# fhausmann/deepgrp

Measured on NVIDIA B200. Metric: bases classified/sec (Mbp/s): value = record resident in HBM (device-timed); e2e = FASTA text in host memory -> TSV text in host memory, higher is better.
Workload: dtype f32

## Files before the change

### deepgrp_b200/csrc/api.cu

```cuda
#include <math.h>
#include <stdarg.h>
#include <string.h>

#include <algorithm>
#include <chrono>
#include <condition_variable>
#include <deque>
#include <mutex>
#include <thread>

#include <cuda_fp16.h>
#include <cmath>

#include "dgrp_internal.cuh"

namespace dgrp {

static thread_local char g_err[1024] = "";

void set_error(const char *fmt, ...) {
  va_list ap;
  va_start(ap, fmt);
  vsnprintf(g_err, sizeof g_err, fmt, ap);
  va_end(ap);
// ... 247 lines not shown
  return DGRP_OK;
}

int dgrp_ctx_synchronize(dgrp_ctx *c) {
  Use use(c->device);
  DGRP_CUDA(cudaStreamSynchronize(c->stream));
  return DGRP_OK;
}
void *dgrp_ctx_stream(dgrp_ctx *c) { return (void *)c->stream; }
int dgrp_ctx_timings(dgrp_ctx *c, dgrp_timings_t *out) { *out = c->timings; return DGRP_OK; }
int64_t dgrp_ctx_launch_count(dgrp_ctx *c) { return c->launches; }

int dgrp_ctx_set_int(dgrp_ctx *c, const char *key, int64_t value) {
  if (!strcmp(key, "mss_chunk")) c->mss_chunk = (int)value;
  else if (!strcmp(key, "mss_max_rounds")) c->mss_max_rounds = (int)value;
  else if (!strcmp(key, "forward_tc")) c->forward_tc = (int)value;
  else if (!strcmp(key, "forward_sum16")) c->forward_sum16 = (int)value;
  else if (!strcmp(key, "forward_fp16x2")) c->forward_fp16x2 = (int)value;
  else if (!strcmp(key, "forward_gather")) c->forward_gather = (int)value;
  else if (!strcmp(key, "forward_fuse_score")) c->forward_fuse_score = (int)value;
  else if (!strcmp(key, "forward_smem_vote")) c->forward_smem_vote = (int)value;
  else if (!strcmp(key, "forward_wide")) c->forward_wide = (int)value;
  else if (!strcmp(key, "forward_overlap")) c->forward_overlap = (int)value;
  else if (!strcmp(key, "forward_ub")) c->forward_ub = (int)value;
  else if (!strcmp(key, "stream_slot_mb")) c->stream_slot_mb = (int)value;
  else if (!strcmp(key, "stream_early_rows")) c->stream_early_rows = (int)value;
  else if (!strcmp(key, "stream_early_slabs")) c->stream_early_slabs = (int)value;
  else if (!strcmp(key, "stream_early_unit")) c->stream_early_unit = (int)value;
  else if (!strcmp(key, "stream_early_ratio")) c->stream_early_ratio = (int)value;
  else if (!strcmp(key, "forward_slab_mb")) c->forward_slab_bytes = (int64_t)value << 20;
  else if (!strcmp(key, "shard_rank")) c->shard_rank = (int)value;
  else if (!strcmp(key, "shard_world")) c->shard_world = (int)value;
  else { set_error("unknown option %s", key); return DGRP_E_ARG; }
  return DGRP_OK;
}
int dgrp_ctx_get_int(dgrp_ctx *c, const char *key, int64_t *value) {
  if (!strcmp(key, "mss_chunk")) *value = c->mss_chunk;
  else if (!strcmp(key, "mss_max_rounds")) *value = c->mss_max_rounds;
  else if (!strcmp(key, "mss_rounds")) *value = c->mss_rounds;
  else if (!strcmp(key, "forward_tc")) *value = c->forward_tc;
  else if (!strcmp(key, "forward_sum16")) *value = c->forward_sum16;
  else if (!strcmp(key, "forward_fp16x2")) *value = c->forward_fp16x2;
  else if (!strcmp(key, "forward_gather")) *value = c->forward_gather;
  else if (!strcmp(key, "forward_fuse_score")) *value = c->forward_fuse_score;
  else if (!strcmp(key, "forward_smem_vote")) *value = c->forward_smem_vote;
  else if (!strcmp(key, "fused_last")) *value = c->fused_last;
  else if (!strcmp(key, "forward_wide")) *value = c->forward_wide;
  else if (!strcmp(key, "forward_overlap")) *value = c->forward_overlap;
  else if (!strcmp(key, "forward_ub")) *value = c->forward_ub;
  else if (!strcmp(key, "stream_slot_mb")) *value = c->stream_slot_mb;
  else if (!strcmp(key, "stream_early_rows")) *value = c->stream_early_rows;
  else if (!strcmp(key, "stream_early_slabs")) *value = c->stream_early_slabs;
  else if (!strcmp(key, "stream_early_unit")) *value = c->stream_early_unit;
  else if (!strcmp(key, "stream_early_ratio")) *value = c->stream_early_ratio;
  else if (!strcmp(key, "stream_early_parts")) *value = c->stream_early_parts;
  else if (!strcmp(key, "forward_slab_mb")) *value = c->forward_slab_bytes >> 20;
  else if (!strcmp(key, "forward_used_tc")) *value = c->forward_used_tc;
  else if (!strcmp(key, "sm_count")) *value = c->sm_count;
  else { set_error("unknown option %s", key); return DGRP_E_ARG; }
  return DGRP_OK;
}


int dgrp_one_hot_stage(dgrp_ctx *c, const uint8_t *seq, int64_t n, int fold_case,
                       int64_t *startpos, int64_t *out_len) {
  Use use(c->device);
  DGRP_REQUIRE(n >= 0, "negative length");
  c->staged_len = -1;
  DGRP_CHECK(c->raw.reserve((size_t)n + 16));
  if (n > 0) DGRP_CUDA(cudaMemcpyAsync(c->raw.p, seq, (size_t)n, cudaMemcpyHostToDevice, c->stream));
  DGRP_CHECK(c->small.reserve(256));
  DGRP_CHECK(c->pin_small.reserve(256));
  int64_t *d_fl = c->small.as<int64_t>() + 16;
  DGRP_CHECK(launch_trim(c, c->raw.as<uint8_t>(), n, fold_case, d_fl));
  int64_t *h = c->pin_small.as<int64_t>() + 8;
  DGRP_CUDA(cudaMemcpyAsync(h, d_fl, 16, cudaMemcpyDeviceToHost, c->stream));
  DGRP_CUDA(cudaStreamSynchronize(c->stream));
  *startpos = h[0];
  *out_len = h[1] - h[0];
  c->staged_n = n; c->staged_start = h[0]; c->staged_len = *out_len;
// ... 1440 lines not shown
```

### deepgrp_b200/csrc/dgrp_internal.cuh

```cuda
#pragma once
#include <cuda_runtime.h>
#include <stdint.h>
#include <stdio.h>
#include <string>
#include <utility>
#include <vector>

#include "../../include/deepgrp_b200.h"

namespace dgrp {

void set_error(const char *fmt, ...);

#define DGRP_CUDA(call)                                                                      \
  do {                                                                                       \
    cudaError_t e__ = (call);                                                                \
    if (e__ != cudaSuccess) {                                                                \
      dgrp::set_error("%s:%d: %s -> %s", __FILE__, __LINE__, #call, cudaGetErrorString(e__)); \
      return DGRP_E_CUDA;                                                                    \
    }                                                                                        \
  } while (0)

#define DGRP_CHECK(call)          \
  do {                            \
// ... 64 lines not shown
      io_a, io_b, io_c, small, segs, rows, mss_a, mss_b, mss_c, mss_d, mss_e, scan, winprobs, gapfill;
  dgrp::PinBuf pin_small, pin_a, pin_b;
  int mss_chunk = 0;
  int mss_max_rounds = 0;
  int mss_rounds = 0;
  int forward_tc = 1;
  int forward_sum16 = 1;
  int forward_fp16x2 = 1;
  int forward_gather = 1;
  int forward_wide = 0;
  int stream_slot_mb = 0;
  int stream_early_rows = 1;
  int stream_early_slabs = 0;
  int stream_early_unit = 0;
  int stream_early_ratio = 0;
  int stream_early_parts = 0;
  int forward_ub = 0;
  int forward_overlap = 1;
  int64_t forward_slab_bytes = (int64_t)8 << 30;
  int forward_smem_vote = 1;
  int forward_fuse_score = 1;
  int fused_last = 0;
  int forward_used_tc = 0;
  std::vector<dgrp_row_t> fa_rows;
  std::vector<int64_t> fa_hdr_off, fa_hdr_len, fa_startpos, fa_length, fa_tsv_off, fa_tsv_len, fa_owner;
  int64_t codes_dev_length = -1, codes_dev_rows = 0;
  uint64_t codes_dev_reserves[2] = {};
  int shard_rank = 0, shard_world = 1;
  dgrp::PinBuf tsv_host;
  int64_t tsv_len = 0;
  dgrp::DevBuf tsv_dev, tsv_prefix;
  dgrp::DevBuf st_raw[2], st_text[2];
  dgrp::PinBuf st_stage[2], st_slot[4];
  int64_t staged_n = 0, staged_start = 0, staged_len = -1;
};

namespace dgrp {

struct Use {
  int prev = -1;
  explicit Use(int dev) {
    cudaGetDevice(&prev);
    if (prev != dev) cudaSetDevice(dev);
    else prev = -1;
  }
  ~Use() {
// ... 58 lines not shown
```

### deepgrp_b200/csrc/forward.cu

```cuda
#include "forward_common.cuh"

namespace dgrp {

Placement make_placement(int64_t length, int T, int step, int batch_size, int compat) {
  Placement p;
  p.step = step;
  const int64_t W = length > T ? (length - T + step - 1) / step : 0;
  p.n_windows = W;
  p.full_windows = W;
  p.tail_base = 0;
  if (compat == DGRP_COMPAT_REFERENCE && batch_size > 0 && W % batch_size != 0) {
    const int64_t nb = W / batch_size, b_last = W % batch_size;
    p.full_windows = nb * batch_size;
    p.tail_base = nb * b_last * (int64_t)step;
  }
  return p;
}


int launch_forward_tc(dgrp_ctx *c, dgrp_model *m, FwdParams &p);
int launch_forward_tcw(dgrp_ctx *c, dgrp_model *m, FwdParams &p, int which);

template <int UP, int RNN = 0>
struct Cfg {
// ... 248 lines not shown

int run_forward_vote(dgrp_ctx *c, dgrp_model *m, const uint8_t *d_codes, int64_t codes_base,
                     int64_t w_begin, int64_t w_end, const Placement &pl, float *d_pred,
                     int64_t pred_row0, int64_t pred_rows, uint8_t *d_label, float *d_score, bool *fused,
                     int64_t w2_begin, int64_t w2_end) {
  if (fused) *fused = false;
  bool has2 = w2_end > w2_begin;
  if (has2 && w_end <= w_begin) { w_begin = w2_begin; w_end = w2_end; has2 = false; }
  auto second = [&]() -> int {
    return has2 ? run_forward_vote(c, m, d_codes, codes_base, w2_begin, w2_end, pl, d_pred, pred_row0, pred_rows) : DGRP_OK;
  };
  FwdParams p = {};
  fill_model(p, m);
  p.codes = d_codes; p.codes_base = codes_base;
  p.w_begin = w_begin; p.w_end = w_end;
  p.step = pl.step; p.full_windows = pl.full_windows; p.tail_base = pl.tail_base;
  p.pred = d_pred; p.pred_row0 = pred_row0; p.pred_rows = pred_rows;
  if (w_end <= w_begin) {
    if (fused && pred_rows > 0)
      DGRP_CUDA(cudaMemsetAsync(d_pred, 0, (size_t)pred_rows * m->C * sizeof(float), c->stream));
    return DGRP_OK;
  }
  c->forward_used_tc = 0;
  if (c->forward_tc) {
    auto dispatch = [&](FwdParams &q, int *used) -> int {
      int rc = DGRP_E_UNSUPPORTED;
      if (c->forward_wide == 0) { rc = launch_forward_tc(c, m, q); *used = 1; }
      if (rc == DGRP_E_UNSUPPORTED && c->forward_wide != 2) { rc = launch_forward_tcw(c, m, q, 1); *used = 2; }
      if (rc == DGRP_E_UNSUPPORTED) { rc = launch_forward_tcw(c, m, q, 2); *used = 3; }
      return rc;
    };
    bool smem_vote = false;
    if (w_end > w_begin) {
      FwdParams q = p;
      q.query = 1;
      int used = 0;
      smem_vote = dispatch(q, &used) == DGRP_OK && q.smem_vote;
    }
    const int64_t per_win = (int64_t)m->T * m->C * (int64_t)sizeof(float);
    int64_t slab = c->forward_slab_bytes / per_win;
    slab = slab < 4096 ? 4096 : slab & ~(int64_t)4095;
    p.win_probs = nullptr;
    if (c->forward_gather && !smem_vote) {
      const int64_t nw = w_end - w_begin < slab ? w_end - w_begin : slab;
      if (nw > 0 && c->winprobs.reserve((size_t)(nw * per_win)) == DGRP_OK) p.win_probs = c->winprobs.as<float>();
      else cudaGetLastError();
// ... 73 lines not shown
```

### deepgrp_b200/csrc/forward_tc.cu

```cuda
#include "forward_tc_common.cuh"

namespace dgrp {

template <int UP, int NP>
struct TCfg {
  static constexpr int NG = 3 * UP;
  static constexpr int N = 3 * UP + 16;
  static constexpr int ROWS = 128, WT = 64;
  static constexpr int UPT = UP / 4;
  static constexpr bool FOLD = NP == 2;
  static constexpr int KP = UP + (FOLD ? 16 : 0);
  static constexpr int KC = KP / 8;
  static constexpr int SBO = KC * 128;
  static constexpr int A_BYTES = ROWS * KP * 2;
  static constexpr int B_BYTES = N * KP * 2;
  static constexpr int PSTRIDE = 3 * UP + 4;
  static constexpr int TCOLS = N <= 64 ? 64 : (N <= 128 ? 128 : 256);
};


template <int UP, typename ST, int NP>
__global__ void __launch_bounds__(TC_THREADS, 1) gru_tc_attention_vote_kernel(const FwdParams p) {
  using K = TCfg<UP, NP>;
  extern __shared__ __align__(128) unsigned char smem_raw[];
  unsigned char *s_B = smem_raw;
  unsigned char *s_A = s_B + NP * K::B_BYTES;
  float *s_P = reinterpret_cast<float *>(s_A + 2 * NP * K::A_BYTES);
  float *s_bh = s_P + 10 * K::PSTRIDE;
  float *s_scale = s_bh + UP;
  float *s_score = s_scale + UP;
  uint8_t *s_codes = reinterpret_cast<uint8_t *>(s_score + (size_t)p.wpp * p.T);
  __shared__ __align__(8) unsigned long long s_ready[2], s_done[2];
  __shared__ uint32_t s_tmem;

  const int tid = threadIdx.x, lane = tid & 31, warp = tid >> 5;
  const int T = p.T;

  {
    const uint4 *src = reinterpret_cast<const uint4 *>(p.Bsplit);
    uint4 *dst = reinterpret_cast<uint4 *>(s_B);
    for (int i = tid; i < NP * K::B_BYTES / 16; i += TC_THREADS) dst[i] = src[i];
    for (int i = tid; i < 10 * K::PSTRIDE; i += TC_THREADS) {
      const int row = i / K::PSTRIDE, j = i % K::PSTRIDE;
      const int c = row >= 8 ? 4 : (row >= 4 ? 7 - row : row);
      float v = 0.f;
      if (j < 2 * UP) v = (p.P[c * 3 * UP + j] + p.b1[j]) * kNegLog2e;
      else if (j < 3 * UP) v = p.P[c * 3 * UP + j] * kTwoLog2e;
      s_P[i] = v;
    }
    for (int i = tid; i < UP; i += TC_THREADS) {
      s_bh[i] = p.b1[2 * UP + i] * kTwoLog2e;
      s_scale[i] = (p.attention && i < p.U) ? p.scale[i] : 0.f;
    }
  }
  if (warp == 0) {
    asm volatile("tcgen05.alloc.cta_group::1.sync.aligned.shared::cta.b32 [%0], %1;" ::"r"(
                     smem_u32(&s_tmem)),
                 "r"(2 * K::TCOLS)
                 : "memory");
    asm volatile("tcgen05.relinquish_alloc_permit.cta_group::1.sync.aligned;" ::: "memory");
  }
#ifdef DGRP_TC_TRACE
  for (int i = tid; i < 17 * 2 * 8; i += TC_THREADS) (&s_tc_trace[0][0][0])[i] = 0u;
  for (int i = tid; i < 16 * 8; i += TC_THREADS) (&s_tc_trace2[0][0])[i] = 0u;
#endif
  if (tid == 0) {
    mbar_init(smem_u32(&s_ready[0]), TC_GATE_WARPS * 32);
    mbar_init(smem_u32(&s_ready[1]), TC_GATE_WARPS * 32);
    mbar_init(smem_u32(&s_done[0]), 1);
    mbar_init(smem_u32(&s_done[1]), 1);
    asm volatile("fence.mbarrier_init.release.cluster;" ::: "memory");
  }
  fence_async_smem();
  tc_fence_before();
  __syncthreads();
  tc_fence_after();
  const uint32_t tmem_base = s_tmem;
  const bool is_gate = warp < TC_GATE_WARPS;
  const int extra = (T & 1) ? 0 : 1;
  const uint32_t bar_ready = smem_u32(&s_ready[0]), bar_done = smem_u32(&s_done[0]);
  const int64_t n_tiles = launch_tiles(p, K::WT);
  const int64_t tile_lo = n_tiles * blockIdx.x / gridDim.x, tile_hi = n_tiles * (blockIdx.x + 1) / gridDim.x;
  const int64_t my_tiles = tile_hi - tile_lo;
  const int lead = my_tiles >= 32 ? (int)(blockIdx.x & 3) : (my_tiles >= 16 ? (int)(blockIdx.x & 1) : 0);
  const uint32_t ab_fmt = NP == 3 ? 1u : 0u;
  const uint32_t idesc = (1u << 4) | (ab_fmt << 7) | (ab_fmt << 10) | ((uint32_t)(K::N >> 3) << 17) |
                         ((uint32_t)(128 >> 4) << 24);

  if (!is_gate) {
    asm volatile("setmaxnreg.dec.sync.aligned.u32 %0;" ::"n"(TC_AUX_REGS));
    if (warp != TC_GATE_WARPS) return;
    int unit = 0;
    for (int64_t tile = tile_lo; tile < tile_hi; ++unit) {
      const int nt = (unit < lead || tile + 1 >= tile_hi) ? 1 : 2;
      const bool live1 = nt == 2;
      TC_TRACE_DECL;
      for (int k = 0; k <= T + extra; ++k) {
#pragma unroll
        for (int s = 0; s < 2; ++s) {
          if (s == 1 && !live1) continue;
          TC_TRACE(6);
          mbar_wait_backoff(bar_ready + 8 * s, (uint32_t)(k & 1));
          tc_fence_after();
          TC_TRACE(5);
          if (lane == 0) {
            const uint32_t a0 = smem_u32(s_A + (size_t)s * NP * K::A_BYTES), b0 = smem_u32(s_B);
            const uint32_t d = tmem_base + (uint32_t)(s * K::TCOLS);
            const int pa[6] = {NP == 3 ? 2 : 1, 0, NP == 3 ? 1 : 0, 1, 0, 0};
            const int pb[6] = {0, NP == 3 ? 2 : 1, NP == 3 ? 1 : 0, 0, 1, 0};
            uint32_t acc = 0;
#pragma unroll
            for (int q = 0; q < (NP == 3 ? 6 : 3); ++q) {
              const int nkc = UP / 16 + ((K::FOLD && pa[q] == 0) ? 1 : 0);
#pragma unroll
              for (int kc = 0; kc < UP / 16 + 1; ++kc) {
                if (kc >= nkc) break;
                const uint64_t ad = umma_desc(a0 + pa[q] * K::A_BYTES + kc * 256, 128, K::SBO);
                const uint64_t bd = umma_desc(b0 + pb[q] * K::B_BYTES + kc * 256, 128, K::SBO);
                umma_bf16(d, ad, bd, idesc, acc);
                acc = 1;
              }
            }
            umma_commit(bar_done + 8 * s);
          }
          __syncwarp();
        }
      }
      tile += nt;
    }
#ifdef DGRP_TC_TRACE
    __syncwarp();
    if (blockIdx.x == 0 && lane < 16) g_tc_trace[16][lane >> 3][lane & 7] += s_tc_trace[16][lane >> 3][lane & 7];
#endif
    return;
  }

  asm volatile("setmaxnreg.inc.sync.aligned.u32 %0;" ::"n"(TC_GATE_REGS));
  ST *sum0 = reinterpret_cast<ST *>(p.scratch) + (size_t)blockIdx.x * 2 * K::WT * T * UP;
  float *proj0 = p.ff2 + (size_t)blockIdx.x * 2 * K::WT * T * 16;
  float *q0 = p.qbuf + (size_t)blockIdx.x * 2 * K::WT * UP;
  const float2 us = make_float2(p.b_unscale, p.b_unscale);
  int unit = 0;
  for (int64_t tile = tile_lo; tile < tile_hi; ++unit) {
    const int nt = (unit < lead || tile + 1 >= tile_hi) ? 1 : 2;
    const bool live1 = nt == 2;
    {
    const int quad = warp & 3, uq = warp >> 2;
    const int row = quad * 32 + lane;
    const int wl = row >> 1, dir = row & 1;
    const float *tblp = s_P + uq * K::UPT;
    const float *bhp = s_bh + uq * K::UPT;
    const uint32_t a_off = (uint32_t)((row >> 3) * K::SBO + (row & 7) * 16 + ((uq * K::UPT) >> 3) * 128);
    const size_t sum_thr = ((size_t)(wl / p.wpp) * T * (UP / 8) * p.wpp + (size_t)(wl % p.wpp)) * 8 + (dir ? 4 : 0);
    const uint32_t oh_off = (uint32_t)((row >> 3) * K::SBO + (row & 7) * 16 + (UP / 8) * 128);
    const uint32_t t_lane = tmem_base + ((uint32_t)(quad * 32) << 16);
    const int full_span = (K::WT - 1) * p.step + T;
    const int cbase = dir * p.code_span + (dir ? full_span - wl * p.step - T : wl * p.step);
    {
      const int nthr = TC_GATE_WARPS * 32;
      for (int s = 0; s < nt; ++s) {
        const TileRange tr = tile_range(p, tile + s, K::WT);
        const int64_t w_first = tr.w0;
        int64_t w_last = w_first + K::WT - 1;
        w_last = w_last < tr.hi ? w_last : tr.hi - 1;
        const int span = (int)((w_last - w_first) * p.step) + T;
        const uint8_t *src = p.codes + (w_first * (int64_t)p.step - p.codes_base);
        uint8_t *fwd_copy = s_codes + (size_t)(2 * s) * p.code_span, *rc_copy = fwd_copy + p.code_span;
        for (int i = tid; i < full_span; i += nthr) {
// ... 128 lines not shown
        }
        TC_TRACE(6);
      }
    }
#pragma unroll
    for (int s = 0; s < 2; ++s) {
      if (s == 1 && !live1) continue;
      mbar_wait(bar_done + 8 * s, (uint32_t)((T + extra) & 1));
      tc_fence_after();
      float pj[4];
      tmem_ld4(t_lane + (uint32_t)(s * K::TCOLS + K::NG + 4 * uq), pj);
      tmem_ld_wait();
      float4 o;
      o.x = pj[0] + __shfl_xor_sync(0xffffffffu, pj[0], 1);
      o.y = pj[1] + __shfl_xor_sync(0xffffffffu, pj[1], 1);
      o.z = pj[2] + __shfl_xor_sync(0xffffffffu, pj[2], 1);
      o.w = pj[3] + __shfl_xor_sync(0xffffffffu, pj[3], 1);
      if (NP == 2) { o.x *= us.x; o.y *= us.x; o.z *= us.x; o.w *= us.x; }
      if (dir == 0)
        *reinterpret_cast<float4 *>(proj0 + ((size_t)(s * K::WT + wl) * T + (T - 1)) * 16 + 4 * uq) = o;
    }
    tc_fence_before();
    }
    __threadfence_block();
    gate_bar_sync();
#pragma unroll 1
    for (int s = 0; s < nt; ++s)
      attention_vote_sum_tile<UP, K::WT, TC_GATE_WARPS, ST>(
          p, sum0 + (size_t)s * K::WT * T * UP, q0 + (size_t)s * K::WT * UP,
          proj0 + (size_t)s * K::WT * T * 16, tile_range(p, tile + s, K::WT), p.wpp, s_scale, s_score,
          p.smem_vote == 1 ? reinterpret_cast<float *>(s_A)
                           : (p.smem_vote == 2 ? reinterpret_cast<float *>(s_codes + 4 * (size_t)p.code_span) : nullptr));
    tile += nt;
  }

  tc_fence_before();
  gate_bar_sync();
#ifdef DGRP_TC_TRACE
  if (blockIdx.x == 0 && tid < 16 * 16) g_tc_trace[tid >> 4][(tid >> 3) & 1][tid & 7] += s_tc_trace[tid >> 4][(tid >> 3) & 1][tid & 7];
  if (blockIdx.x == 0 && tid < 16 * 8) g_tc_trace2[tid >> 3][tid & 7] += s_tc_trace2[tid >> 3][tid & 7];
#endif
  if (warp == 0) {
    asm volatile("tcgen05.dealloc.cta_group::1.sync.aligned.b32 %0, %1;" ::"r"(tmem_base),
                 "r"(2 * K::TCOLS)
                 : "memory");
  }
// ... 2 lines not shown
template <int UP, int NP>
static size_t tc_smem_bytes(int T, int wpp, int code_span) {
  using K = TCfg<UP, NP>;
  return (size_t)NP * K::B_BYTES + 2 * NP * K::A_BYTES +
         sizeof(float) * ((size_t)10 * K::PSTRIDE + 2 * UP + (size_t)wpp * T) + 4 * (size_t)code_span + 128;
}

template <int UP, typename ST, int NP>
static int launch_tc_t(dgrp_ctx *c, dgrp_model *m, FwdParams &p) {
  using K = TCfg<UP, NP>;
  const int64_t n_windows = p.w_end - p.w_begin;
  if (n_windows <= 0 && p.w2_end <= p.w2_begin) return DGRP_OK;
  const int64_t span = (int64_t)(K::WT - 1) * p.step + p.T;
  if (span > 16384) return DGRP_E_UNSUPPORTED;
  p.code_span = (int)((span + 15) & ~(int64_t)15);
  int wpp = K::WT;
  while (wpp > 8 && tc_smem_bytes<UP, NP>(p.T, wpp, p.code_span) > 227 * 1024) wpp >>= 1;
  const size_t smem = tc_smem_bytes<UP, NP>(p.T, wpp, p.code_span);
  if (smem > 227 * 1024) return DGRP_E_UNSUPPORTED;
  p.wpp = wpp;
  const size_t vote_bytes = (size_t)span * p.C * sizeof(float);
  size_t smem_total = smem;
  p.smem_vote = 0;
  if (c->forward_smem_vote) {
    if (vote_bytes <= (size_t)2 * NP * K::A_BYTES) p.smem_vote = 1;
    else if (smem + vote_bytes <= 227 * 1024) { p.smem_vote = 2; smem_total = smem + vote_bytes; }
  }
  if (p.query) return DGRP_OK;
  if (p.smem_vote) p.win_probs = nullptr;
  auto kern = gru_tc_attention_vote_kernel<UP, ST, NP>;
  DGRP_CUDA(cudaFuncSetAttribute(kern, cudaFuncAttributeMaxDynamicSharedMemorySize, (int)smem_total));
  const int64_t n_tiles = (n_windows > 0 ? (n_windows + K::WT - 1) / K::WT : 0) +
                          (p.w2_end > p.w2_begin ? (p.w2_end - p.w2_begin + K::WT - 1) / K::WT : 0);
  const int64_t n_pairs = (n_tiles + 1) / 2;
  const int grid = (int)(n_pairs < c->sm_count ? n_pairs : c->sm_count);
  const size_t rows = (size_t)grid * 2 * K::WT;
  DGRP_CHECK(c->avg.reserve(rows * p.T * UP * sizeof(ST) + rows * UP * sizeof(float)));
  DGRP_CHECK(c->io_c.reserve(rows * p.T * 16 * sizeof(float)));
  p.scratch = c->avg.as<float>();
  p.qbuf = reinterpret_cast<float *>(c->avg.as<unsigned char>() + rows * p.T * UP * sizeof(ST));
  p.ff2 = c->io_c.as<float>();
  kern<<<grid, TC_THREADS, smem_total, c->stream>>>(p);
  c->launches++;
  DGRP_CUDA(cudaGetLastError());
  return DGRP_OK;
}

#ifdef DGRP_TC_TRACE
extern "C" int dgrp_debug_tc_trace(unsigned long long *out, int reset) {
  if (reset) {
    static unsigned long long zero[17][2][8];
    return (int)cudaMemcpyToSymbol(g_tc_trace, zero, sizeof(zero));
  }
  return (int)cudaMemcpyFromSymbol(out, g_tc_trace, sizeof(unsigned long long) * 17 * 2 * 8);
}
extern "C" int dgrp_debug_tc_trace2(unsigned long long *out, int reset) {
  if (reset) {
    static unsigned long long zero[16][8];
    return (int)cudaMemcpyToSymbol(g_tc_trace2, zero, sizeof(zero));
  }
  return (int)cudaMemcpyFromSymbol(out, g_tc_trace2, sizeof(unsigned long long) * 16 * 8);
}
#endif

template <int UP>
static int launch_tc_up(dgrp_ctx *c, dgrp_model *m, FwdParams &p) {
// ... 18 lines not shown
```

### deepgrp_b200/csrc/forward_tc_common.cuh

```cuda
#pragma once
#include <cuda_bf16.h>
#include <cuda_fp16.h>

#include "forward_common.cuh"

namespace dgrp {

constexpr int TC_GATE_WARPS = 16;
constexpr int TC_THREADS = (TC_GATE_WARPS + 4) * 32;
constexpr int TC_GATE_REGS = 112, TC_AUX_REGS = 24;
constexpr float kNegLog2e = -1.4426950408889634f;
constexpr float kTwoLog2e = 2.8853900817779268f;

#ifdef DGRP_TC_TRACE
static __device__ unsigned long long g_tc_trace[17][2][8];
__shared__ unsigned int s_tc_trace[17][2][8];
#define TC_TRACE_DECL unsigned int tr_t = (unsigned int)clock64()
#define TC_TRACE(seg)                                                         \
  do {                                                                        \
    const unsigned int now__ = (unsigned int)clock64();                       \
    if (lane == 0) atomicAdd(&s_tc_trace[warp][s][seg], now__ - tr_t);        \
    tr_t = now__;                                                             \
  } while (0)
#define TC_TRACE2(seg)                                                        \
  do {                                                                        \
    const unsigned int now__ = (unsigned int)clock64();                       \
    if (lane == 0) atomicAdd(&s_tc_trace2[warp][seg], now__ - tr_t);          \
    tr_t = now__;                                                             \
  } while (0)
__shared__ unsigned int s_tc_trace2[16][8];
static __device__ unsigned long long g_tc_trace2[16][8];
#else
#define TC_TRACE_DECL
// ... 189 lines not shown
}
__device__ __forceinline__ void ldg256(const float *p, float (&v)[8]) {
  asm volatile("ld.global.v8.f32 {%0,%1,%2,%3,%4,%5,%6,%7}, [%8];"
               : "=f"(v[0]), "=f"(v[1]), "=f"(v[2]), "=f"(v[3]), "=f"(v[4]), "=f"(v[5]), "=f"(v[6]), "=f"(v[7])
               : "l"(p));
}
__device__ __forceinline__ float tanh_mufu(float x) {
  float y;
  asm("tanh.approx.f32 %0, %1;" : "=f"(y) : "f"(x));
  return y;
}
__device__ __forceinline__ float exp_fast(float x) {
  return ex2_approx(x * 1.4426950408889634f);
}
__device__ __forceinline__ float inv4_dot(const float *d, const float *sc) {
  const float2 d01 = make_float2(d[0], d[1]), d23 = make_float2(d[2], d[3]);
  const float2 m = __fmul2_rn(d01, d23);
  const float inv = rcp_approx(m.x * m.y);
  const float2 j = make_float2(inv * m.y, inv * m.x);
  const float2 i01 = __fmul2_rn(j, d23), i23 = __fmul2_rn(j, d01);
  return fmaf(sc[0], i01.x, fmaf(sc[1], i01.y, fmaf(sc[2], i23.x, sc[3] * i23.y)));
}

template <int UP, int WT, int NWARPS, typename ST>
__device__ __forceinline__ void attention_vote_sum_tile(const FwdParams &p, const ST *sum, const float *qbuf,
                                                        const float *proj, const TileRange tr, int wpp,
                                                        const float *s_scale, float *s_score, float *s_vote = nullptr) {
  const int64_t w_tile0 = tr.w0;
  const int tid = threadIdx.x, warp = tid >> 5, lane = tid & 31;
  const int T = p.T, C = p.C;
  const int vspan = (WT - 1) * p.step + T;
  if (s_vote) {
    for (int i = tid; i < vspan * C; i += NWARPS * 32) s_vote[i] = 0.f;
  }
  constexpr int NCH = UP / 8;
  constexpr int CPL = NCH / 4;
  constexpr int CH = CPL > 2 ? 2 : CPL;
  constexpr bool H16 = sizeof(ST) == 2;
  constexpr int NV = H16 ? 1 : 2;
  constexpr int UNR = H16 ? 4 : 2;
  constexpr int PU = 11;
  TC_TRACE_DECL;
  for (int w0 = 0; w0 < WT; w0 += wpp) {
    if (w_tile0 + w0 >= tr.hi) break;
    if (p.attention) {
      const int ngrp = wpp >> 3, grp = warp % ngrp, sl = warp / ngrp, nsl = NWARPS / ngrp;
      const int wi = lane & 7, cj = lane >> 3;
      const int wl = w0 + grp * 8 + wi;
      const int t_begin = (int)((int64_t)T * sl / nsl), t_end = (int)((int64_t)T * (sl + 1) / nsl);
#pragma unroll 1
      for (int i0 = 0; i0 < CPL; i0 += CH) {
      float q2[CH][8], sc2[CH][8];
#pragma unroll
      for (int i = 0; i < CH; ++i) {
        const int u0 = (cj + 4 * (i0 + i)) * 8;
#pragma unroll
        for (int j = 0; j < 8; ++j) {
          q2[i][j] = H16 ? qbuf[(size_t)wl * UP + u0 + j] : qbuf[(size_t)wl * UP + u0 + j] * kTwoLog2e;
          sc2[i][j] = H16 ? s_scale[u0 + j] : -2.0f * s_scale[u0 + j];
        }
      }
      const ST *sum_pass = sum + (size_t)(w0 / wpp) * T * NCH * wpp * 8;
      const ST *base = sum_pass + ((size_t)(cj + 4 * i0) * wpp + (grp * 8 + wi)) * 8;
      constexpr int PF_BLOCK = 4, PF_AHEAD = 12;
      const uint32_t ROW_BYTES = (uint32_t)(NCH * wpp * 8 * sizeof(ST));
      if (grp == 0 && lane == 0 && i0 == 0) {
        const int n0 = min(PF_AHEAD, t_end - t_begin);
        l2_prefetch(sum_pass + (size_t)t_begin * NCH * wpp * 8, (uint32_t)n0 * ROW_BYTES);
      }
      for (int t0 = t_begin; t0 < t_end; t0 += UNR) {
        if (grp == 0 && lane == 0 && i0 == 0 && (t0 - t_begin) % PF_BLOCK == 0) {
          const int ta = t0 + PF_AHEAD;
          if (ta < t_end) l2_prefetch(sum_pass + (size_t)ta * NCH * wpp * 8, (uint32_t)min(PF_BLOCK, t_end - ta) * ROW_BYTES);
        }
        uint4 v[UNR][CH][NV];
#pragma unroll
        for (int k = 0; k < UNR; ++k) {
          const int t = min(t0 + k, t_end - 1);
#pragma unroll
          for (int i = 0; i < CH; ++i)
#pragma unroll
            for (int n = 0; n < NV; ++n)
              v[k][i][n] = __ldcs(reinterpret_cast<const uint4 *>(base + ((size_t)t * NCH + 4 * i) * wpp * 8) + n);
        }
#pragma unroll
        for (int k = 0; k < UNR; ++k) {
          float sacc = 0.f;
#pragma unroll
          for (int i = 0; i < CH; ++i) {
            float x[8];
            if (H16) {
              const uint32_t wv[4] = {v[k][i][0].x, v[k][i][0].y, v[k][i][0].z, v[k][i][0].w};
#pragma unroll
              for (int j = 0; j < 4; ++j) {
                const float2 f = __half22float2(*reinterpret_cast<const __half2 *>(&wv[j]));
                x[2 * j] = f.x; x[2 * j + 1] = f.y;
              }
            } else {
              const uint32_t wv[8] = {v[k][i][0].x, v[k][i][0].y, v[k][i][0].z, v[k][i][0].w,
                                      v[k][i][NV - 1].x, v[k][i][NV - 1].y, v[k][i][NV - 1].z, v[k][i][NV - 1].w};
#pragma unroll
              for (int j = 0; j < 8; ++j) x[j] = __uint_as_float(wv[j]);
            }
            if (H16) {
#pragma unroll
              for (int j = 0; j < 8; ++j) sacc = fmaf(sc2[i][j], tanh_mufu(fmaf(x[j], 0.5f, q2[i][j])), sacc);
            } else {
              float d[8];
#pragma unroll
              for (int j = 0; j < 8; ++j)
                d[j] = ex2_approx(fminf(fmaf(x[j], 1.4426950408889634f, q2[i][j]), 30.0f)) + 1.0f;
              sacc += inv4_dot(d, sc2[i]) + inv4_dot(d + 4, sc2[i] + 4);
            }
          }
          sacc += __shfl_xor_sync(0xffffffffu, sacc, 8);
          sacc += __shfl_xor_sync(0xffffffffu, sacc, 16);
          if (cj == 0 && t0 + k < t_end) {
            float *dst = s_score + (size_t)(grp * 8 + wi) * T + t0 + k;
            *dst = (CH < CPL && i0 > 0) ? *dst + sacc : sacc;
          }
        }
      }
      }
    }
    if (lane == 0 && warp < wpp) l2_prefetch(proj + (size_t)(w0 + warp) * T * 16, (uint32_t)T * 64u);
    TC_TRACE2(0);
    asm volatile("bar.sync 1, %0;" ::"n"(NWARPS * 32) : "memory");
    TC_TRACE2(1);
    for (int wq = warp; wq < wpp; wq += NWARPS) {
      const int wl = w0 + wq;
      if (lane == 0 && wq + NWARPS < wpp)
        l2_prefetch(proj + (size_t)(wl + NWARPS) * T * 16, (uint32_t)T * 64u);
      const int64_t w = w_tile0 + wl;
      if (w >= tr.hi) break;
      const float *pr = proj + (size_t)wl * T * 16;
      const float *sc = s_score + (size_t)wq * T;
      float ctxk[5] = {0.f, 0.f, 0.f, 0.f, 0.f};
      if (p.attention) {
        float m_run = -INFINITY, l_run = 0.f, cacc[5] = {0.f, 0.f, 0.f, 0.f, 0.f};
        for (int t0 = lane; t0 < T; t0 += 32 * PU) {
          float sv[PU], k1[PU][5];
#pragma unroll
          for (int k = 0; k < PU; ++k) {
            const int t = t0 + 32 * k;
            const bool ok = t < T;
            float row[8] = {0.f, 0.f, 0.f, 0.f, 0.f, 0.f, 0.f, 0.f};
            if (ok) ldg256(pr + (size_t)t * 16, row);
#pragma unroll
            for (int c = 0; c < 5; ++c) k1[k][c] = row[c];
            sv[k] = ok ? sc[t] : -INFINITY;
          }
          float m_new = m_run;
#pragma unroll
          for (int k = 0; k < PU; ++k) m_new = fmaxf(m_new, sv[k]);
          if (m_new > -INFINITY) {
            const float corr = exp_fast(m_run - m_new);
            l_run *= corr;
#pragma unroll
            for (int c = 0; c < 5; ++c) cacc[c] *= corr;
#pragma unroll
            for (int k = 0; k < PU; ++k) {
              const float e = exp_fast(sv[k] - m_new);
              l_run += e;
#pragma unroll
              for (int c = 0; c < 5; ++c) cacc[c] = fmaf(e, k1[k][c], cacc[c]);
            }
            m_run = m_new;
          }
        }
        float m_all = m_run;
        for (int off = 16; off > 0; off >>= 1) m_all = fmaxf(m_all, __shfl_xor_sync(0xffffffffu, m_all, off));
        const float f = (m_run == -INFINITY) ? 0.f : exp_fast(m_run - m_all);
        float l = l_run * f;
#pragma unroll
        for (int c = 0; c < 5; ++c) cacc[c] *= f;
        for (int off = 16; off > 0; off >>= 1) {
          l += __shfl_xor_sync(0xffffffffu, l, off);
#pragma unroll
          for (int c = 0; c < 5; ++c) cacc[c] += __shfl_xor_sync(0xffffffffu, cacc[c], off);
        }
#pragma unroll
        for (int c = 0; c < 5; ++c) ctxk[c] = cacc[c] / l;
      }
      TC_TRACE2(2);
      const int64_t place = (w < p.full_windows ? w * (int64_t)p.step
                                                : p.tail_base + (w - p.full_windows) * (int64_t)p.step) -
                            p.pred_row0;
      float cb[5];
#pragma unroll
      for (int c = 0; c < 5; ++c) cb[c] = c < C ? ctxk[c] + p.ffb[c] : 0.f;
      for (int t0 = lane; t0 < T; t0 += 32 * PU) {
        float k2[PU][5];
#pragma unroll
        for (int k = 0; k < PU; ++k) {
          const int t = t0 + 32 * k;
          const bool ok = t < T;
          float row[8] = {0.f, 0.f, 0.f, 0.f, 0.f, 0.f, 0.f, 0.f};
          if (ok) ldg256(pr + (size_t)t * 16 + 8, row);
#pragma unroll
          for (int c = 0; c < 5; ++c) k2[k][c] = row[c];
        }
#pragma unroll
        for (int k = 0; k < PU; ++k) {
          const int t = t0 + 32 * k;
          float lg[5], mx = -INFINITY;
#pragma unroll
          for (int c = 0; c < 5; ++c) {
            lg[c] = c < C ? k2[k][c] + cb[c] : -INFINITY;
            mx = fmaxf(mx, lg[c]);
          }
          float sum_e = 0.f;
#pragma unroll
          for (int c = 0; c < 5; ++c) { lg[c] = c < C ? exp_fast(lg[c] - mx) : 0.f; sum_e += lg[c]; }
          const float inv = 1.0f / sum_e;
          if (s_vote && w < p.full_windows) {
            if (t < T) {
              int *dst = reinterpret_cast<int *>(s_vote) + ((int)(w - w_tile0) * p.step + t) * C;
#pragma unroll
              for (int c = 0; c < 5; ++c)
                if (c < C) atomicMax(dst + c, __float_as_int(lg[c] * inv));
            }
          } else if (p.win_probs) {
            if (t < T) {
              float *dst = p.win_probs + ((size_t)(w - p.w_begin) * T + t) * C;
#pragma unroll
              for (int c = 0; c < 5; ++c)
                if (c < C) dst[c] = lg[c] * inv;
            }
          } else {
            const int64_t r = place + t;
            if (t < T && r >= 0 && r < p.pred_rows) {
              int *dst = reinterpret_cast<int *>(p.pred + (size_t)r * C);
#pragma unroll
              for (int c = 0; c < 5; ++c)
                if (c < C) atomicMax(dst + c, __float_as_int(lg[c] * inv));
            }
          }
        }
      }
    }
    TC_TRACE2(3);
    asm volatile("bar.sync 1, %0;" ::"n"(NWARPS * 32) : "memory");
    TC_TRACE2(4);
  }
  if (s_vote) {
    const int64_t row0 = w_tile0 * (int64_t)p.step - p.pred_row0;
    const int64_t tail_lo = p.tail_base - p.pred_row0;
    const int64_t w_max = p.w2_end > p.w2_begin && p.w2_end > p.w_end ? p.w2_end : p.w_end;
    const int64_t tail_hi = tail_lo + (w_max > p.full_windows ? (w_max - p.full_windows - 1) * (int64_t)p.step + T : 0);
    const bool first = w_tile0 == tr.lo;
    const bool last = w_tile0 + WT >= (p.full_windows < tr.hi ? p.full_windows : tr.hi);
    const int own_lo = first ? 0 : T - p.step;
    const int own_hi = last ? vspan : WT * p.step;
    for (int r = tid; r < vspan; r += NWARPS * 32) {
      const int64_t g = row0 + r;
      if (g < 0 || g >= p.pred_rows) continue;
      float v[5];
      bool any = false;
#pragma unroll
      for (int c = 0; c < 5; ++c) { v[c] = c < C ? s_vote[r * C + c] : 0.f; any |= v[c] != 0.f; }
      if (!any) continue;
      float *dst = p.pred + (size_t)g * C;
      const bool shared_row = r < own_lo || r >= own_hi || (g >= tail_lo && g < tail_hi);
      if (shared_row) {
#pragma unroll
        for (int c = 0; c < 5; ++c)
          if (c < C) atomicMax(reinterpret_cast<int *>(dst) + c, __float_as_int(v[c]));
      } else {
#pragma unroll
        for (int c = 0; c < 5; ++c)
          if (c < C) dst[c] = v[c];
      }
    }
    asm volatile("bar.sync 1, %0;" ::"n"(NWARPS * 32) : "memory");
  }
}

}
```

Before: 580.4.

## Offload attention/vote of first tile to async warps via mbarrier ring

Adds an async mode, on by default, where three auxiliary warps compute the attention and vote epilogue for the first tile of each pair. They run against double-buffered scratch slots synchronised through full/empty mbarriers, while the gate warps handle the second tile and move on to the next GRU unit. The aux warps use a lean variant with fewer live registers and a shared-memory ring vote buffer that is flushed incrementally. Registers are rebalanced between gate and aux warps, and scratch memory doubles. The aim is to hide epilogue latency behind tensor-core GRU work, at the cost of fewer gate registers and more complex synchronisation.

```diff
diff --git a/deepgrp_b200/csrc/api.cu b/deepgrp_b200/csrc/api.cu
--- a/deepgrp_b200/csrc/api.cu
+++ b/deepgrp_b200/csrc/api.cu
@@ -293,6 +293,7 @@
   else if (!strcmp(key, "forward_smem_vote")) c->forward_smem_vote = (int)value;
   else if (!strcmp(key, "forward_wide")) c->forward_wide = (int)value;
   else if (!strcmp(key, "forward_overlap")) c->forward_overlap = (int)value;
+  else if (!strcmp(key, "forward_async_attention")) c->forward_async_attention = (int)value;
   else if (!strcmp(key, "forward_ub")) c->forward_ub = (int)value;
   else if (!strcmp(key, "stream_slot_mb")) c->stream_slot_mb = (int)value;
   else if (!strcmp(key, "stream_early_rows")) c->stream_early_rows = (int)value;
@@ -318,6 +319,7 @@
   else if (!strcmp(key, "fused_last")) *value = c->fused_last;
   else if (!strcmp(key, "forward_wide")) *value = c->forward_wide;
   else if (!strcmp(key, "forward_overlap")) *value = c->forward_overlap;
+  else if (!strcmp(key, "forward_async_attention")) *value = c->forward_async_attention;
   else if (!strcmp(key, "forward_ub")) *value = c->forward_ub;
   else if (!strcmp(key, "stream_slot_mb")) *value = c->stream_slot_mb;
   else if (!strcmp(key, "stream_early_rows")) *value = c->stream_early_rows;
@@ -327,6 +329,7 @@
   else if (!strcmp(key, "stream_early_parts")) *value = c->stream_early_parts;
   else if (!strcmp(key, "forward_slab_mb")) *value = c->forward_slab_bytes >> 20;
   else if (!strcmp(key, "forward_used_tc")) *value = c->forward_used_tc;
+  else if (!strcmp(key, "forward_used_async")) *value = c->forward_used_async;
   else if (!strcmp(key, "sm_count")) *value = c->sm_count;
   else { set_error("unknown option %s", key); return DGRP_E_ARG; }
   return DGRP_OK;
diff --git a/deepgrp_b200/csrc/dgrp_internal.cuh b/deepgrp_b200/csrc/dgrp_internal.cuh
--- a/deepgrp_b200/csrc/dgrp_internal.cuh
+++ b/deepgrp_b200/csrc/dgrp_internal.cuh
@@ -110,6 +110,8 @@
   int forward_fuse_score = 1;
   int fused_last = 0;
   int forward_used_tc = 0;
+  int forward_async_attention = 1;
+  int forward_used_async = 0;
   std::vector<dgrp_row_t> fa_rows;
   std::vector<int64_t> fa_hdr_off, fa_hdr_len, fa_startpos, fa_length, fa_tsv_off, fa_tsv_len, fa_owner;
   int64_t codes_dev_length = -1, codes_dev_rows = 0;
diff --git a/deepgrp_b200/csrc/forward.cu b/deepgrp_b200/csrc/forward.cu
--- a/deepgrp_b200/csrc/forward.cu
+++ b/deepgrp_b200/csrc/forward.cu
@@ -294,6 +294,7 @@
     return DGRP_OK;
   }
   c->forward_used_tc = 0;
+  c->forward_used_async = 0;
   if (c->forward_tc) {
     auto dispatch = [&](FwdParams &q, int *used) -> int {
       int rc = DGRP_E_UNSUPPORTED;
diff --git a/deepgrp_b200/csrc/forward_tc.cu b/deepgrp_b200/csrc/forward_tc.cu
--- a/deepgrp_b200/csrc/forward_tc.cu
+++ b/deepgrp_b200/csrc/forward_tc.cu
@@ -19,7 +19,7 @@
 };
 
 
-template <int UP, typename ST, int NP>
+template <int UP, typename ST, int NP, bool ASYNC>
 __global__ void __launch_bounds__(TC_THREADS, 1) gru_tc_attention_vote_kernel(const FwdParams p) {
   using K = TCfg<UP, NP>;
   extern __shared__ __align__(128) unsigned char smem_raw[];
@@ -32,6 +32,7 @@
   uint8_t *s_codes = reinterpret_cast<uint8_t *>(s_score + (size_t)p.wpp * p.T);
   __shared__ __align__(8) unsigned long long s_ready[2], s_done[2];
   __shared__ uint32_t s_tmem;
+  __shared__ __align__(8) unsigned long long s_full[2], s_empty[2];
 
   const int tid = threadIdx.x, lane = tid & 31, warp = tid >> 5;
   const int T = p.T;
@@ -69,6 +70,12 @@
     mbar_init(smem_u32(&s_ready[1]), TC_GATE_WARPS * 32);
     mbar_init(smem_u32(&s_done[0]), 1);
     mbar_init(smem_u32(&s_done[1]), 1);
+    if (ASYNC) {
+      mbar_init(smem_u32(&s_full[0]), TC_GATE_WARPS * 32);
+      mbar_init(smem_u32(&s_full[1]), TC_GATE_WARPS * 32);
+      mbar_init(smem_u32(&s_empty[0]), TC_ATT_WARPS * 32);
+      mbar_init(smem_u32(&s_empty[1]), TC_ATT_WARPS * 32);
+    }
     asm volatile("fence.mbarrier_init.release.cluster;" ::: "memory");
   }
   fence_async_smem();
@@ -82,14 +89,36 @@
   const int64_t n_tiles = launch_tiles(p, K::WT);
   const int64_t tile_lo = n_tiles * blockIdx.x / gridDim.x, tile_hi = n_tiles * (blockIdx.x + 1) / gridDim.x;
   const int64_t my_tiles = tile_hi - tile_lo;
-  const int lead = my_tiles >= 32 ? (int)(blockIdx.x & 3) : (my_tiles >= 16 ? (int)(blockIdx.x & 1) : 0);
+  const int lead = ASYNC ? 0 : (my_tiles >= 32 ? (int)(blockIdx.x & 3) : (my_tiles >= 16 ? (int)(blockIdx.x & 1) : 0));
   const uint32_t ab_fmt = NP == 3 ? 1u : 0u;
   const uint32_t idesc = (1u << 4) | (ab_fmt << 7) | (ab_fmt << 10) | ((uint32_t)(K::N >> 3) << 17) |
                          ((uint32_t)(128 >> 4) << 24);
 
+  const uint32_t bar_full = smem_u32(&s_full[0]), bar_empty = smem_u32(&s_empty[0]);
+
   if (!is_gate) {
-    asm volatile("setmaxnreg.dec.sync.aligned.u32 %0;" ::"n"(TC_AUX_REGS));
-    if (warp != TC_GATE_WARPS) return;
+    asm volatile("setmaxnreg.dec.sync.aligned.u32 %0;" ::"n"(ASYNC ? TC_AUX_REGS_ASYNC : TC_AUX_REGS));
+    if (warp != TC_GATE_WARPS) {
+      if (ASYNC) {
+        const int ring = (p.wpp - 1) * p.step + T;
+        float *s_ring = p.smem_vote ? reinterpret_cast<float *>(s_codes + 4 * (size_t)p.code_span) : nullptr;
+        if (s_ring)
+          for (int i = tid - TC_ATT_WARP0 * 32; i < ring * p.C; i += TC_ATT_WARPS * 32) s_ring[i] = 0.f;
+        int unit = 0;
+        for (int64_t tile = tile_lo; tile < tile_hi; ++unit) {
+          const int nt = (unit < lead || tile + 1 >= tile_hi) ? 1 : 2;
+          const int set = unit & 1;
+          mbar_wait(bar_full + 8 * set, (uint32_t)((unit >> 1) & 1));
+          const size_t slot = (size_t)set * gridDim.x + blockIdx.x;
+          attention_vote_sum_tile<UP, K::WT, TC_ATT_WARPS, ST, 2, TC_ATT_WARP0, true>(
+              p, reinterpret_cast<const ST *>(p.scratch) + slot * 2 * K::WT * T * UP, p.qbuf + slot * 2 * K::WT * UP,
+              p.ff2 + slot * 2 * K::WT * T * 16, tile_range(p, tile, K::WT), p.wpp, s_scale, s_score, s_ring, ring);
+          mbar_arrive(bar_empty + 8 * set);
+          tile += nt;
+        }
+      }
+      return;
+    }
     int unit = 0;
     for (int64_t tile = tile_lo; tile < tile_hi; ++unit) {
       const int nt = (unit < lead || tile + 1 >= tile_hi) ? 1 : 2;
@@ -135,15 +164,18 @@
     return;
   }
 
-  asm volatile("setmaxnreg.inc.sync.aligned.u32 %0;" ::"n"(TC_GATE_REGS));
-  ST *sum0 = reinterpret_cast<ST *>(p.scratch) + (size_t)blockIdx.x * 2 * K::WT * T * UP;
-  float *proj0 = p.ff2 + (size_t)blockIdx.x * 2 * K::WT * T * 16;
-  float *q0 = p.qbuf + (size_t)blockIdx.x * 2 * K::WT * UP;
+  asm volatile("setmaxnreg.inc.sync.aligned.u32 %0;" ::"n"(ASYNC ? TC_GATE_REGS_ASYNC : TC_GATE_REGS));
   const float2 us = make_float2(p.b_unscale, p.b_unscale);
   int unit = 0;
   for (int64_t tile = tile_lo; tile < tile_hi; ++unit) {
     const int nt = (unit < lead || tile + 1 >= tile_hi) ? 1 : 2;
     const bool live1 = nt == 2;
+    const int set = ASYNC ? (unit & 1) : 0;
+    const size_t slot = (size_t)set * gridDim.x + blockIdx.x;
+    ST *sum0 = reinterpret_cast<ST *>(p.scratch) + slot * 2 * K::WT * T * UP;
+    float *proj0 = p.ff2 + slot * 2 * K::WT * T * 16;
+    float *q0 = p.qbuf + slot * 2 * K::WT * UP;
+    if (ASYNC && unit >= 2) mbar_wait(bar_empty + 8 * set, (uint32_t)(((unit >> 1) - 1) & 1));
     {
     const int quad = warp & 3, uq = warp >> 2;
     const int row = quad * 32 + lane;
@@ -318,6 +350,23 @@
     }
     tc_fence_before();
     }
+    if (ASYNC) {
+      mbar_arrive(bar_full + 8 * (unit & 1));
+      if (live1) {
+        const int vote_bytes = ((K::WT - 1) * p.step + T) * p.C * (int)sizeof(float);
+        const bool vote_in_a = vote_bytes + p.wpp * T * (int)sizeof(float) <= 2 * NP * K::A_BYTES;
+        const int score_off = vote_in_a ? (vote_bytes + 15) & ~15 : 0;
+        __threadfence_block();
+        gate_bar_sync();
+        attention_vote_sum_tile<UP, K::WT, TC_GATE_WARPS, ST>(
+            p, sum0 + (size_t)K::WT * T * UP, q0 + (size_t)K::WT * UP, proj0 + (size_t)K::WT * T * 16,
+            tile_range(p, tile + 1, K::WT), p.wpp, s_scale, reinterpret_cast<float *>(s_A + score_off),
+            vote_in_a ? reinterpret_cast<float *>(s_A) : nullptr);
+        gate_bar_sync();
+      }
+      tile += nt;
+      continue;
+    }
     __threadfence_block();
     gate_bar_sync();
 #pragma unroll 1
@@ -366,19 +415,27 @@
   const size_t vote_bytes = (size_t)span * p.C * sizeof(float);
   size_t smem_total = smem;
   p.smem_vote = 0;
-  if (c->forward_smem_vote) {
+  const int ring = 7 * p.step + p.T;
+  const size_t smem_async = tc_smem_bytes<UP, NP>(p.T, 8, p.code_span) + (size_t)ring * p.C * sizeof(float);
+  const bool async = c->forward_async_attention && c->forward_smem_vote && smem_async <= 227 * 1024 &&
+                     (size_t)8 * p.T * sizeof(float) <= (size_t)2 * NP * K::A_BYTES;
+  if (async) {
+    p.wpp = 8;
+    p.smem_vote = 3;
+    smem_total = smem_async;
+  } else if (c->forward_smem_vote) {
     if (vote_bytes <= (size_t)2 * NP * K::A_BYTES) p.smem_vote = 1;
     else if (smem + vote_bytes <= 227 * 1024) { p.smem_vote = 2; smem_total = smem + vote_bytes; }
   }
   if (p.query) return DGRP_OK;
   if (p.smem_vote) p.win_probs = nullptr;
-  auto kern = gru_tc_attention_vote_kernel<UP, ST, NP>;
+  auto kern = async ? gru_tc_attention_vote_kernel<UP, ST, NP, true> : gru_tc_attention_vote_kernel<UP, ST, NP, false>;
   DGRP_CUDA(cudaFuncSetAttribute(kern, cudaFuncAttributeMaxDynamicSharedMemorySize, (int)smem_total));
   const int64_t n_tiles = (n_windows > 0 ? (n_windows + K::WT - 1) / K::WT : 0) +
                           (p.w2_end > p.w2_begin ? (p.w2_end - p.w2_begin + K::WT - 1) / K::WT : 0);
   const int64_t n_pairs = (n_tiles + 1) / 2;
   const int grid = (int)(n_pairs < c->sm_count ? n_pairs : c->sm_count);
-  const size_t rows = (size_t)grid * 2 * K::WT;
+  const size_t rows = (size_t)grid * 2 * K::WT * (async ? 2 : 1);
   DGRP_CHECK(c->avg.reserve(rows * p.T * UP * sizeof(ST) + rows * UP * sizeof(float)));
   DGRP_CHECK(c->io_c.reserve(rows * p.T * 16 * sizeof(float)));
   p.scratch = c->avg.as<float>();
@@ -386,6 +443,7 @@
   p.ff2 = c->io_c.as<float>();
   kern<<<grid, TC_THREADS, smem_total, c->stream>>>(p);
   c->launches++;
+  c->forward_used_async = async ? 1 : 0;
   DGRP_CUDA(cudaGetLastError());
   return DGRP_OK;
 }
diff --git a/deepgrp_b200/csrc/forward_tc_common.cuh b/deepgrp_b200/csrc/forward_tc_common.cuh
--- a/deepgrp_b200/csrc/forward_tc_common.cuh
+++ b/deepgrp_b200/csrc/forward_tc_common.cuh
@@ -9,6 +9,9 @@
 constexpr int TC_GATE_WARPS = 16;
 constexpr int TC_THREADS = (TC_GATE_WARPS + 4) * 32;
 constexpr int TC_GATE_REGS = 112, TC_AUX_REGS = 24;
+constexpr int TC_ATT_WARPS = 3, TC_ATT_WARP0 = TC_GATE_WARPS + 1;
+constexpr int TC_GATE_REGS_ASYNC = 104, TC_AUX_REGS_ASYNC = 64;
+static_assert(TC_GATE_WARPS * 32 * TC_GATE_REGS_ASYNC + 4 * 32 * TC_AUX_REGS_ASYNC == TC_THREADS * 96, "register pool");
 constexpr float kNegLog2e = -1.4426950408889634f;
 constexpr float kTwoLog2e = 2.8853900817779268f;
 
@@ -244,15 +247,59 @@
   return fmaf(sc[0], i01.x, fmaf(sc[1], i01.y, fmaf(sc[2], i23.x, sc[3] * i23.y)));
 }
 
-template <int UP, int WT, int NWARPS, typename ST>
+template <int WT, int NWARPS, bool RING>
+__device__ __forceinline__ void vote_flush_rows(const FwdParams &p, float *s_vote, const TileRange tr, int r_lo, int r_hi,
+                                                int ring, int tid) {
+  const int T = p.T, C = p.C;
+  const int64_t w_tile0 = tr.w0;
+  const int vspan = (WT - 1) * p.step + T;
+  const int64_t row0 = w_tile0 * (int64_t)p.step - p.pred_row0;
+  const int64_t tail_lo = p.tail_base - p.pred_row0;
+  const int64_t w_max = p.w2_end > p.w2_begin && p.w2_end > p.w_end ? p.w2_end : p.w_end;
+  const int64_t tail_hi = tail_lo + (w_max > p.full_windows ? (w_max - p.full_windows - 1) * (int64_t)p.step + T : 0);
+  const bool first = w_tile0 == tr.lo;
+  const bool last = w_tile0 + WT >= (p.full_windows < tr.hi ? p.full_windows : tr.hi);
+  const int own_lo = first ? 0 : T - p.step;
+  const int own_hi = last ? vspan : WT * p.step;
+  for (int r = r_lo + tid; r < r_hi; r += NWARPS * 32) {
+    const int64_t g = row0 + r;
+    if (!RING && (g < 0 || g >= p.pred_rows)) continue;
+    float *slot = s_vote + (RING ? r % ring : r) * C;
+    float v[5];
+    bool any = false;
+#pragma unroll
+    for (int c = 0; c < 5; ++c) { v[c] = c < C ? slot[c] : 0.f; any |= v[c] != 0.f; }
+    if (RING) {
+#pragma unroll
+      for (int c = 0; c < 5; ++c)
+        if (c < C) slot[c] = 0.f;
+      if (g < 0 || g >= p.pred_rows) continue;
+    }
+    if (!any) continue;
+    float *dst = p.pred + (size_t)g * C;
+    const bool shared_row = r < own_lo || r >= own_hi || (g >= tail_lo && g < tail_hi);
+    if (shared_row) {
+#pragma unroll
+      for (int c = 0; c < 5; ++c)
+        if (c < C) atomicMax(reinterpret_cast<int *>(dst) + c, __float_as_int(v[c]));
+    } else {
+#pragma unroll
+      for (int c = 0; c < 5; ++c)
+        if (c < C) dst[c] = v[c];
+    }
+  }
+}
+
+template <int UP, int WT, int NWARPS, typename ST, int BAR = 1, int W0 = 0, bool LEAN = false>
 __device__ __forceinline__ void attention_vote_sum_tile(const FwdParams &p, const ST *sum, const float *qbuf,
                                                         const float *proj, const TileRange tr, int wpp,
-                                                        const float *s_scale, float *s_score, float *s_vote = nullptr) {
+                                                        const float *s_scale, float *s_score, float *s_vote = nullptr,
+                                                        int ring = 0) {
   const int64_t w_tile0 = tr.w0;
-  const int tid = threadIdx.x, warp = tid >> 5, lane = tid & 31;
+  const int tid = threadIdx.x - W0 * 32, warp = tid >> 5, lane = tid & 31;
   const int T = p.T, C = p.C;
   const int vspan = (WT - 1) * p.step + T;
-  if (s_vote) {
+  if (s_vote && !LEAN) {
     for (int i = tid; i < vspan * C; i += NWARPS * 32) s_vote[i] = 0.f;
   }
   constexpr int NCH = UP / 8;
@@ -260,8 +307,9 @@
   constexpr int CH = CPL > 2 ? 2 : CPL;
   constexpr bool H16 = sizeof(ST) == 2;
   constexpr int NV = H16 ? 1 : 2;
-  constexpr int UNR = H16 ? 4 : 2;
+  constexpr int UNR = LEAN ? (H16 ? 2 : 1) : (H16 ? 4 : 2);
   constexpr int PU = 11;
+  constexpr int PUV = LEAN ? 4 : PU;
   TC_TRACE_DECL;
   for (int w0 = 0; w0 < WT; w0 += wpp) {
     if (w_tile0 + w0 >= tr.hi) break;
@@ -279,7 +327,7 @@
 #pragma unroll
         for (int j = 0; j < 8; ++j) {
           q2[i][j] = H16 ? qbuf[(size_t)wl * UP + u0 + j] : qbuf[(size_t)wl * UP + u0 + j] * kTwoLog2e;
-          sc2[i][j] = H16 ? s_scale[u0 + j] : -2.0f * s_scale[u0 + j];
+          if (!LEAN) sc2[i][j] = H16 ? s_scale[u0 + j] : -2.0f * s_scale[u0 + j];
         }
       }
       const ST *sum_pass = sum + (size_t)(w0 / wpp) * T * NCH * wpp * 8;
@@ -325,14 +373,23 @@
               for (int j = 0; j < 8; ++j) x[j] = __uint_as_float(wv[j]);
             }
             if (H16) {
-#pragma unroll
-              for (int j = 0; j < 8; ++j) sacc = fmaf(sc2[i][j], tanh_mufu(fmaf(x[j], 0.5f, q2[i][j])), sacc);
+              const float *scl = s_scale + (cj + 4 * (i0 + i)) * 8;
+#pragma unroll
+              for (int j = 0; j < 8; ++j)
+                sacc = fmaf(LEAN ? scl[j] : sc2[i][j], tanh_mufu(fmaf(x[j], 0.5f, q2[i][j])), sacc);
             } else {
               float d[8];
 #pragma unroll
               for (int j = 0; j < 8; ++j)
                 d[j] = ex2_approx(fminf(fmaf(x[j], 1.4426950408889634f, q2[i][j]), 30.0f)) + 1.0f;
-              sacc += inv4_dot(d, sc2[i]) + inv4_dot(d + 4, sc2[i] + 4);
+              if (LEAN) {
+                float scl[8];
+#pragma unroll
+                for (int j = 0; j < 8; ++j) scl[j] = -2.0f * s_scale[(cj + 4 * (i0 + i)) * 8 + j];
+                sacc += inv4_dot(d, scl) + inv4_dot(d + 4, scl + 4);
+              } else {
+                sacc += inv4_dot(d, sc2[i]) + inv4_dot(d + 4, sc2[i] + 4);
+              }
             }
           }
           sacc += __shfl_xor_sync(0xffffffffu, sacc, 8);
@@ -347,7 +404,7 @@
     }
     if (lane == 0 && warp < wpp) l2_prefetch(proj + (size_t)(w0 + warp) * T * 16, (uint32_t)T * 64u);
     TC_TRACE2(0);
-    asm volatile("bar.sync 1, %0;" ::"n"(NWARPS * 32) : "memory");
+    asm volatile("bar.sync %0, %1;" ::"n"(BAR), "n"(NWARPS * 32) : "memory");
     TC_TRACE2(1);
     for (int wq = warp; wq < wpp; wq += NWARPS) {
       const int wl = w0 + wq;
@@ -361,33 +418,57 @@
       if (p.attention) {
         float m_run = -INFINITY, l_run = 0.f, cacc[5] = {0.f, 0.f, 0.f, 0.f, 0.f};
         for (int t0 = lane; t0 < T; t0 += 32 * PU) {
-          float sv[PU], k1[PU][5];
-#pragma unroll
-          for (int k = 0; k < PU; ++k) {
-            const int t = t0 + 32 * k;
-            const bool ok = t < T;
-            float row[8] = {0.f, 0.f, 0.f, 0.f, 0.f, 0.f, 0.f, 0.f};
-            if (ok) ldg256(pr + (size_t)t * 16, row);
-#pragma unroll
-            for (int c = 0; c < 5; ++c) k1[k][c] = row[c];
-            sv[k] = ok ? sc[t] : -INFINITY;
-          }
-          float m_new = m_run;
-#pragma unroll
-          for (int k = 0; k < PU; ++k) m_new = fmaxf(m_new, sv[k]);
-          if (m_new > -INFINITY) {
-            const float corr = exp_fast(m_run - m_new);
-            l_run *= corr;
-#pragma unroll
-            for (int c = 0; c < 5; ++c) cacc[c] *= corr;
+          if constexpr (LEAN) {
+            float m_new = m_run;
+#pragma unroll
+            for (int k = 0; k < PU; ++k) m_new = fmaxf(m_new, t0 + 32 * k < T ? sc[t0 + 32 * k] : -INFINITY);
+            if (m_new > -INFINITY) {
+              const float corr = exp_fast(m_run - m_new);
+              l_run *= corr;
+#pragma unroll
+              for (int c = 0; c < 5; ++c) cacc[c] *= corr;
+#pragma unroll
+              for (int k = 0; k < PU; ++k) {
+                const int t = t0 + 32 * k;
+                const bool ok = t < T;
+                float row[8] = {0.f, 0.f, 0.f, 0.f, 0.f, 0.f, 0.f, 0.f};
+                if (ok) ldg256(pr + (size_t)t * 16, row);
+                const float e = exp_fast((ok ? sc[t] : -INFINITY) - m_new);
+                l_run += e;
+#pragma unroll
+                for (int c = 0; c < 5; ++c) cacc[c] = fmaf(e, row[c], cacc[c]);
+              }
+              m_run = m_new;
+            }
+          } else {
+            float sv[PU], k1[PU][5];
 #pragma unroll
             for (int k = 0; k < PU; ++k) {
-              const float e = exp_fast(sv[k] - m_new);
-              l_run += e;
-#pragma unroll
-              for (int c = 0; c < 5; ++c) cacc[c] = fmaf(e, k1[k][c], cacc[c]);
-            }
-            m_run = m_new;
+              const int t = t0 + 32 * k;
+              const bool ok = t < T;
+              float row[8] = {0.f, 0.f, 0.f, 0.f, 0.f, 0.f, 0.f, 0.f};
+              if (ok) ldg256(pr + (size_t)t * 16, row);
+#pragma unroll
+              for (int c = 0; c < 5; ++c) k1[k][c] = row[c];
+              sv[k] = ok ? sc[t] : -INFINITY;
+            }
+            float m_new = m_run;
+#pragma unroll
+            for (int k = 0; k < PU; ++k) m_new = fmaxf(m_new, sv[k]);
+            if (m_new > -INFINITY) {
+              const float corr = exp_fast(m_run - m_new);
+              l_run *= corr;
+#pragma unroll
+              for (int c = 0; c < 5; ++c) cacc[c] *= corr;
+#pragma unroll
+              for (int k = 0; k < PU; ++k) {
+                const float e = exp_fast(sv[k] - m_new);
+                l_run += e;
+#pragma unroll
+                for (int c = 0; c < 5; ++c) cacc[c] = fmaf(e, k1[k][c], cacc[c]);
+              }
+              m_run = m_new;
+            }
           }
         }
         float m_all = m_run;
@@ -411,10 +492,11 @@
       float cb[5];
 #pragma unroll
       for (int c = 0; c < 5; ++c) cb[c] = c < C ? ctxk[c] + p.ffb[c] : 0.f;
-      for (int t0 = lane; t0 < T; t0 += 32 * PU) {
-        float k2[PU][5];
-#pragma unroll
-        for (int k = 0; k < PU; ++k) {
+      const int vslot = LEAN && s_vote ? (int)(w - w_tile0) * p.step % ring : 0;
+      for (int t0 = lane; t0 < T; t0 += 32 * PUV) {
+        float k2[PUV][5];
+#pragma unroll
+        for (int k = 0; k < PUV; ++k) {
           const int t = t0 + 32 * k;
           const bool ok = t < T;
           float row[8] = {0.f, 0.f, 0.f, 0.f, 0.f, 0.f, 0.f, 0.f};
@@ -423,7 +505,7 @@
           for (int c = 0; c < 5; ++c) k2[k][c] = row[c];
         }
 #pragma unroll
-        for (int k = 0; k < PU; ++k) {
+        for (int k = 0; k < PUV; ++k) {
           const int t = t0 + 32 * k;
           float lg[5], mx = -INFINITY;
 #pragma unroll
@@ -437,7 +519,9 @@
           const float inv = 1.0f / sum_e;
           if (s_vote && w < p.full_windows) {
             if (t < T) {
-              int *dst = reinterpret_cast<int *>(s_vote) + ((int)(w - w_tile0) * p.step + t) * C;
+              int slot = LEAN ? vslot + t : (int)(w - w_tile0) * p.step + t;
+              if (LEAN && slot >= ring) slot -= ring;
+              int *dst = reinterpret_cast<int *>(s_vote) + slot * C;
 #pragma unroll
               for (int c = 0; c < 5; ++c)
                 if (c < C) atomicMax(dst + c, __float_as_int(lg[c] * inv));
@@ -462,39 +546,16 @@
       }
     }
     TC_TRACE2(3);
-    asm volatile("bar.sync 1, %0;" ::"n"(NWARPS * 32) : "memory");
+    asm volatile("bar.sync %0, %1;" ::"n"(BAR), "n"(NWARPS * 32) : "memory");
     TC_TRACE2(4);
+    if (LEAN && s_vote) {
+      const bool more = w0 + wpp < WT && w_tile0 + w0 + wpp < tr.hi;
+      vote_flush_rows<WT, NWARPS, true>(p, s_vote, tr, w0 * p.step, more ? (w0 + wpp) * p.step : vspan, ring, tid);
+    }
   }
-  if (s_vote) {
-    const int64_t row0 = w_tile0 * (int64_t)p.step - p.pred_row0;
-    const int64_t tail_lo = p.tail_base - p.pred_row0;
-    const int64_t w_max = p.w2_end > p.w2_begin && p.w2_end > p.w_end ? p.w2_end : p.w_end;
-    const int64_t tail_hi = tail_lo + (w_max > p.full_windows ? (w_max - p.full_windows - 1) * (int64_t)p.step + T : 0);
-    const bool first = w_tile0 == tr.lo;
-    const bool last = w_tile0 + WT >= (p.full_windows < tr.hi ? p.full_windows : tr.hi);
-    const int own_lo = first ? 0 : T - p.step;
-    const int own_hi = last ? vspan : WT * p.step;
-    for (int r = tid; r < vspan; r += NWARPS * 32) {
-      const int64_t g = row0 + r;
-      if (g < 0 || g >= p.pred_rows) continue;
-      float v[5];
-      bool any = false;
-#pragma unroll
-      for (int c = 0; c < 5; ++c) { v[c] = c < C ? s_vote[r * C + c] : 0.f; any |= v[c] != 0.f; }
-      if (!any) continue;
-      float *dst = p.pred + (size_t)g * C;
-      const bool shared_row = r < own_lo || r >= own_hi || (g >= tail_lo && g < tail_hi);
-      if (shared_row) {
-#pragma unroll
-        for (int c = 0; c < 5; ++c)
-          if (c < C) atomicMax(reinterpret_cast<int *>(dst) + c, __float_as_int(v[c]));
-      } else {
-#pragma unroll
-        for (int c = 0; c < 5; ++c)
-          if (c < C) dst[c] = v[c];
-      }
-    }
-    asm volatile("bar.sync 1, %0;" ::"n"(NWARPS * 32) : "memory");
+  if (s_vote && !LEAN) {
+    vote_flush_rows<WT, NWARPS, false>(p, s_vote, tr, 0, vspan, 0, tid);
+    asm volatile("bar.sync %0, %1;" ::"n"(BAR), "n"(NWARPS * 32) : "memory");
   }
 }
 
```

Result: slower. 569.4 (median of 6 runs) (-1.9%).
